# marcin-ochman/modular-slam

Measured on AMD Instinct MI355X. Metric: ORB keypoints extracted+matched /sec, 640×480 RGB-D, 1/2/4/8 GPU; HBM GB/s vs roofline, higher is better.
Workload: dtype u8

## Files before the change

### modular-slam_amd/csrc/k_quadtree.hip

```cpp
#include "common.hpp"
#include <cstdlib>

namespace mslam
{

constexpr int QT = 512;
constexpr int kSmallKp = 512, kSmallQT = 256;
constexpr int kMidKp = 1024, kMidQT = 512;
constexpr int kLdsKp = 2048;
constexpr int kMaxCellsPerLevel = 2048;
constexpr int kBigNodes = 4096;
constexpr int kBigKp = 12288;
constexpr int kBigMinPixels = 400000;
constexpr int kMaxInitNodes = 64;
constexpr int kMaxPasses = 40;

struct Scan
{
    uint32_t wsum[QT / 64];
};

__device__ __forceinline__ uint32_t wave_incl_scan(uint32_t v)
{
    int x = (int)v;
    x += __builtin_amdgcn_update_dpp(0, x, 0x111, 0xF, 0xF, true);
    x += __builtin_amdgcn_update_dpp(0, x, 0x112, 0xF, 0xF, true);
    x += __builtin_amdgcn_update_dpp(0, x, 0x114, 0xF, 0xE, true);
    x += __builtin_amdgcn_update_dpp(0, x, 0x118, 0xF, 0xC, true);
    x += __builtin_amdgcn_update_dpp(0, x, 0x142, 0xA, 0xF, true);
    x += __builtin_amdgcn_update_dpp(0, x, 0x143, 0xC, 0xF, true);
    return (uint32_t)x;
}

template <int NT>
__device__ __forceinline__ uint32_t block_excl_scan(uint32_t v, Scan& s, uint32_t& total)
{
    const int lane = threadIdx.x & 63, wave = threadIdx.x >> 6;
    const uint32_t inc = wave_incl_scan(v);
    if(lane == 63)
        s.wsum[wave] = inc;
    __syncthreads();
    uint32_t base = 0, tot = 0;
#pragma unroll
    for(int w = 0; w < NT / 64; ++w)
    {
        const uint32_t x = s.wsum[w];
        if(w < wave)
// ... 131 lines not shown
    __syncthreads();
    if(tid == 0)
    {
        uint32_t n0 = 0;
        for(int i = 0; i < n_init; ++i)
        {
            init_pos[i] = n0;
            if(init_cnt[i] != 0)
            {
                const int ix = i % lv.nxg, iy = i / lv.nxg;
                nodes[n0] = pack_node((int)(lv.delta_x * ix), (int)(lv.delta_y * iy), (int)(lv.delta_x * (ix + 1)),
                                      (int)(lv.delta_y * (iy + 1)));
                ncnt[n0] = (idx_t)init_cnt[i];
                ++n0;
            }
        }
        sh_n = n0;
    }
    __syncthreads();
    for(uint32_t k = tid; k < N; k += NT)
    {
        const uint32_t idx = kp_node[k];
        if(idx != kNoNode)
            kp_node[k] = (idx_t)init_pos[idx];
    }
    uint32_t n = sh_n;
    __syncthreads();

    const float sf = lv.scale;
    const float min_size_f = (float)a.min_size;
    bool converged = false;
    for(int pass = 0; pass < kMaxPasses && n > 0; ++pass)
    {
        for(uint32_t pos = tid; pos < n; pos += NT)
        {
            int bx, by, ex, ey;
            unpack_node(nodes[pos], bx, by, ex, ey);
            const unsigned area = (unsigned)((ex - bx) * (ey - by));
            const bool keep = (uint32_t)ncnt[pos] == 1u || __fmul_rn(__fmul_rn((float)area, sf), sf) <= min_size_f;
            ninfo[pos] = keep ? 0u : 1u;
            if(!keep)
                S::cc_zero(cc, pos);
        }
        __syncthreads();
        for(uint32_t k = tid; k < N; k += NT)
        {
            const uint32_t pos = kp_node[k];
            if(pos == kNoNode || !(ninfo[pos] & 1u))
                continue;
            int bx, by, ex, ey;
            unpack_node(nodes[pos], bx, by, ex, ey);
            const int cx = bx + ((ex - bx + 1) >> 1), cy = by + ((ey - by + 1) >> 1);
            const uint32_t p = cand[k];
            S::cc_add(cc, pos, (cx <= kp_x(p) ? 1 : 0) + (cy <= kp_y(p) ? 2 : 0));
        }
        __syncthreads();
        uint32_t D = 0, U = 0;
        for(uint32_t base = 0; base < n; base += NT)
        {
            const uint32_t pos = base + tid;
            uint32_t nchild = 0, und = 0, mask = 0, div = 0;
            if(pos < n)
            {
                div = ninfo[pos] & 1u;
                if(div)
                {
                    mask = (S::cc_get(cc, pos, 0) ? 1u : 0u) | (S::cc_get(cc, pos, 1) ? 2u : 0u) |
                           (S::cc_get(cc, pos, 2) ? 4u : 0u) | (S::cc_get(cc, pos, 3) ? 8u : 0u);
                    nchild = (uint32_t)__popc(mask);
                }
                else
                    und = 1;
            }
            uint32_t totD, totU, exD, exU;
            block_excl_scan2<NT>(nchild, und, scan, scan2, exD, exU, totD, totU);
            if(pos < n)
            {
// ... 87 lines not shown
        a.sel_cnt[slot] = n;
    return true;
}

template <int NT>
__device__ __forceinline__ uint32_t quad_cell_offsets(const uint32_t* ccnt, int n_cells, uint32_t* cell_off, Scan& scan)
{
    const int tid = threadIdx.x;
    uint32_t running = 0;
    for(int base = 0; base < n_cells; base += NT)
    {
        const int i = base + tid;
        const uint32_t v = i < n_cells ? ccnt[i] : 0u;
        uint32_t tot;
        const uint32_t ex = block_excl_scan<NT>(v, scan, tot);
        if(i < n_cells)
            cell_off[i] = running + ex;
        running += tot;
    }
    if(tid == 0)
        cell_off[n_cells] = running;
    __syncthreads();
    return running;
}

__device__ __forceinline__ int quad_class(uint32_t N, int n_cells, unsigned classes)
{
    if((classes & 1u) && N <= (uint32_t)kSmallKp && n_cells <= 2 * kSmallKp - 1)
        return 0;
    if((classes & 2u) && N <= (uint32_t)kMidKp && n_cells <= 2 * kMidKp - 1)
        return 1;
    return 2;
}
template <int KP, int NT, int CLS>
__global__ __launch_bounds__(NT) __attribute__((amdgpu_waves_per_eu(CLS == 2 ? 4 : 8))) void k_quadtree(Geometry g, QuadArgs a, unsigned big_levels)
{
    __shared__ Scan scan, scan2;
    __shared__ uint32_t l_cand[KP];
    __shared__ uint2 l_nodes_a[KP], l_nodes_b[KP];
    __shared__ uint32_t l_cc[KP * 2];
    __shared__ uint16_t l_kp_node[KP], l_ncnt_a[KP], l_ncnt_b[KP], l_nbase[KP];
    __shared__ uint8_t l_ninfo[KP];
    __shared__ uint32_t init_cnt[kMaxInitNodes];
    __shared__ uint32_t init_pos[kMaxInitNodes];
    __shared__ uint32_t sh_n;
    constexpr int kCellsFit = 2 * KP - 1;
    static_assert(CLS != 2 || kCellsFit >= kMaxCellsPerLevel, "cell offsets must fit");
    const unsigned classes = big_levels >> 30;
    uint32_t* cell_off = reinterpret_cast<uint32_t*>(l_nodes_b);

    const int level = (int)((blockIdx.x + blockIdx.y) % (unsigned)g.n_levels);
    const size_t frame = blockIdx.y + g.frame0;
    const LevelGeom& lv = g.lv[level];
    const int tid = threadIdx.x;
    const size_t slot = frame * g.n_levels + level;
    const size_t cap = (size_t)a.cand_cap;
    uint32_t* cand = a.cand + slot * cap;
    uint32_t* sel = a.sel + slot * cap;

    const int n_cells = lv.n_cells;
    if(n_cells > kCellsFit)
        return;
    const uint32_t* ccnt = a.cell_cnt + frame * g.n_cells + lv.cell_base;
    const uint32_t N = quad_cell_offsets<NT>(ccnt, n_cells, cell_off, scan);
    if(quad_class(N, n_cells, classes) != CLS)
        return;
    if(N > (uint32_t)a.cand_cap)
    {
        if(tid == 0)
        {
            atomicOr(a.flags, kFlagCandOverflow);
            a.cand_cnt[slot] = 0;
            a.sel_cnt[slot] = 0;
        }
        return;
    }
    if(tid == 0)
        a.cand_cnt[slot] = N;
    if(N == 0)
    {
        if(tid == 0)
            a.sel_cnt[slot] = 0;
        return;
    }
    if(N <= (uint32_t)KP)
        quad_run<LdsStore, NT>(g, a, lv, frame, slot, tid, N, n_cells, cell_off, l_cand, cand, l_kp_node, l_nodes_a, l_nodes_b,
                               l_ncnt_a, l_ncnt_b, l_ninfo, l_nbase, l_cc, l_cc, sel, scan, scan2, init_cnt, init_pos, sh_n);
    else if((big_levels >> level) & 1u)
        return;
    else
        quad_run<GlobalStore, NT>(g, a, lv, frame, slot, tid, N, n_cells, cell_off, cand, cand, a.kp_node + slot * cap,
                                  a.nodes_a + slot * cap, a.nodes_b + slot * cap, a.ncnt_a + slot * cap,
                                  a.ncnt_b + slot * cap, a.ninfo + slot * cap, a.best + slot * cap,
                                  a.child_cnt + slot * cap * 4, a.best + slot * cap, sel, scan, scan2, init_cnt, init_pos,
                                  sh_n);
}

__global__ __launch_bounds__(QT) void k_quadtree_big(Geometry g, QuadArgs a, unsigned big_levels)
{
    extern __shared__ __attribute__((aligned(16))) uint8_t big_lds[];
    __shared__ Scan scan, scan2;
    __shared__ uint32_t init_cnt[kMaxInitNodes];
    __shared__ uint32_t init_pos[kMaxInitNodes];
    __shared__ uint32_t sh_n;
    uint2* l_nodes_a = reinterpret_cast<uint2*>(big_lds);
    uint2* l_nodes_b = l_nodes_a + kBigNodes;
    uint32_t* l_cc = reinterpret_cast<uint32_t*>(l_nodes_b + kBigNodes);
    uint16_t* l_kp_node = reinterpret_cast<uint16_t*>(l_cc + 2 * kBigNodes);
    uint16_t* l_ncnt_a = l_kp_node + kBigKp;
    uint16_t* l_ncnt_b = l_ncnt_a + kBigNodes;
    uint16_t* l_nbase = l_ncnt_b + kBigNodes;
    uint8_t* l_ninfo = reinterpret_cast<uint8_t*>(l_nbase + kBigNodes);
    static_assert(kBigNodes * sizeof(uint2) >= (kMaxCellsPerLevel + 1) * sizeof(uint32_t), "cell offsets must fit");
    uint32_t* cell_off = reinterpret_cast<uint32_t*>(l_nodes_b);

    int level = 0;
    {
        unsigned m = big_levels;
        const unsigned which = (blockIdx.x + blockIdx.y) % gridDim.x;
        for(unsigned i = 0; i < which; ++i)
            m &= m - 1;
        level = __ffs((int)m) - 1;
    }
    const size_t frame = blockIdx.y + g.frame0;
    const LevelGeom& lv = g.lv[level];
    const int tid = threadIdx.x;
    const size_t slot = frame * g.n_levels + level;
    const size_t cap = (size_t)a.cand_cap;
    uint32_t* cand = a.cand + slot * cap;
    uint32_t* sel = a.sel + slot * cap;
    const int n_cells = lv.n_cells;
    const uint32_t* ccnt = a.cell_cnt + frame * g.n_cells + lv.cell_base;
    const uint32_t N = quad_cell_offsets<QT>(ccnt, n_cells, cell_off, scan);
    if(N <= (uint32_t)kLdsKp || N > (uint32_t)a.cand_cap)
        return;
    bool done = false;
    if(N <= (uint32_t)kBigKp)
        done = quad_run<BigStore, QT>(g, a, lv, frame, slot, tid, N, n_cells, cell_off, cand, cand, l_kp_node, l_nodes_a, l_nodes_b,
                                  l_ncnt_a, l_ncnt_b, l_ninfo, l_nbase, l_cc, l_cc, sel, scan, scan2, init_cnt, init_pos, sh_n);
    if(!done)
    {
        __syncthreads();
        quad_cell_offsets<QT>(ccnt, n_cells, cell_off, scan);
        quad_run<GlobalStore, QT>(g, a, lv, frame, slot, tid, N, n_cells, cell_off, cand, cand, a.kp_node + slot * cap,
                              a.nodes_a + slot * cap, a.nodes_b + slot * cap, a.ncnt_a + slot * cap,
                              a.ncnt_b + slot * cap, a.ninfo + slot * cap, a.best + slot * cap,
                              a.child_cnt + slot * cap * 4, a.best + slot * cap, sel, scan, scan2, init_cnt, init_pos,
                              sh_n);
    }
}

void launch_quadtree(const Geometry& g, const QuadArgs& a, int frame0, int n_frames, hipStream_t s)
{
    dim3 grid(g.n_levels, n_frames);
    Geometry gg = g;
    gg.frame0 = frame0;
    unsigned big_levels = 0;
    for(int l = 0; l < g.n_levels; ++l)
        if(g.lv[l].w * g.lv[l].h > kBigMinPixels)
            big_levels |= 1u << l;
    static const unsigned classes_env = [] { const char* e = getenv("MSLAM_HIP_QUAD_CLASSES"); return e ? (unsigned)atoi(e) & 3u : 3u; }();
    const unsigned classes = n_frames < 8 ? 0u : classes_env;
    const unsigned bl = big_levels | (classes << 30);
    hipLaunchKernelGGL((k_quadtree<kLdsKp, QT, 2>), grid, dim3(QT), 0, s, gg, a, bl);
    if(classes & 2u)
        hipLaunchKernelGGL((k_quadtree<kMidKp, kMidQT, 1>), grid, dim3(kMidQT), 0, s, gg, a, bl);
    if(classes & 1u)
        hipLaunchKernelGGL((k_quadtree<kSmallKp, kSmallQT, 0>), grid, dim3(kSmallQT), 0, s, gg, a, bl);
    if(big_levels != 0)
    {
        constexpr size_t lds = (size_t)kBigNodes * (8 + 8 + 8 + 2 + 2 + 2 + 1) + (size_t)kBigKp * 2;
        static const bool attr = [] {
            return hipFuncSetAttribute((const void*)k_quadtree_big, hipFuncAttributeMaxDynamicSharedMemorySize, (int)lds) == hipSuccess;
        }();
        (void)attr;
        hipLaunchKernelGGL(k_quadtree_big, dim3((unsigned)__builtin_popcount(big_levels), n_frames), dim3(QT), lds, s, gg, a,
                           big_levels);
    }
}

}
```

### include/mslam_hip.h

```cpp
#ifndef MSLAM_HIP_H_
#define MSLAM_HIP_H_

#include <stddef.h>
#include <stdint.h>

#ifdef __cplusplus
extern "C" {
#endif

#define MSLAM_HIP_ABI_VERSION 5

enum
{
    MSLAM_HIP_OK = 0,
    MSLAM_HIP_E_INVALID = 1,
    MSLAM_HIP_E_RUNTIME = 2,
    MSLAM_HIP_E_CAPACITY = 3,
    MSLAM_HIP_E_NO_VOCABULARY = 4,
    MSLAM_HIP_E_FORMAT = 5,
    MSLAM_HIP_E_NO_MODEL = 6
};

typedef struct mslam_hip_ctx mslam_hip_ctx;

// ... 259 lines not shown
} mslam_hip_track_result;
int mslam_hip_track(mslam_hip_ctx* ctx, const uint8_t* desc, const float* xy, int n, const uint16_t* depth, int width,
                    int height, float factor, double fx, double fy, double cx, double cy, int ref_id,
                    const int32_t* vote_ids, int n_vote, double ratio, int iterations, double reprojection_error,
                    uint64_t seed, int use_extrinsic_guess, const double* rvec, const double* tvec,
                    int min_matched_points , int new_keyframe_min_landmarks , int new_id ,
                    double z_max , mslam_hip_track_result* out, int32_t* vote_counts ,
                    int32_t* pair_from, int32_t* pair_to, uint8_t* inliers, int pair_stride,
                    int32_t* entry_src, int32_t* entry_kp, int entry_capacity);

typedef mslam_hip_track_result mslam_hip_track_window_result;
int mslam_hip_track_window(mslam_hip_ctx* ctx, const uint8_t* desc, const float* xy, const int32_t* n, int stride,
                           const uint16_t* depth, int S, int width, int height, float factor, double fx, double fy, double cx,
                           double cy, int ref_id, const int32_t* vote_ids, int n_vote, int ref_vote_pos, double ratio,
                           int iterations, double reprojection_error, uint64_t seed, int use_extrinsic_guess,
                           const double* rvec, const double* tvec, int min_matched_points, int new_keyframe_min_landmarks,
                           int new_id, double z_max, mslam_hip_track_window_result* out , int* first_event,
                           int32_t* vote_counts , int32_t* entry_src, int32_t* entry_kp,
                           int entry_capacity);
int mslam_hip_track_window_dev(mslam_hip_ctx* ctx, int first_frame, int n_frames, double fx, double fy, double cx, double cy,
                               int ref_id, const int32_t* vote_ids, int n_vote, int ref_vote_pos, double ratio, int iterations,
                               double reprojection_error, uint64_t seed, int use_extrinsic_guess, const double* rvec,
                               const double* tvec, int min_matched_points, int new_keyframe_min_landmarks, int new_id,
                               double z_max, mslam_hip_track_window_result* out , int* first_event,
                               int32_t* vote_counts, int32_t* entry_src, int32_t* entry_kp, int entry_capacity);

enum
{
    MSLAM_HIP_DBG_PYRAMID = 0,
    MSLAM_HIP_DBG_BLURRED = 1,
    MSLAM_HIP_DBG_CANDIDATES = 2,
    MSLAM_HIP_DBG_SELECTED = 3,
    MSLAM_HIP_DBG_CELLS = 4,
    MSLAM_HIP_DBG_FORMS = 5
};
int mslam_hip_level_geometry(mslam_hip_ctx* ctx, int* widths, int* heights, float* scales);
int mslam_hip_debug_read(mslam_hip_ctx* ctx, int what, int frame, int level, void* dst, size_t dst_bytes,
                         size_t* n_items);

int mslam_hip_debug_counts(mslam_hip_ctx* ctx, int what, int32_t* out, int n_frames);

int mslam_hip_copy_to_host(mslam_hip_ctx* ctx, void* dst_host, const void* src_dev, size_t bytes);

int mslam_hip_set_profiling(mslam_hip_ctx* ctx, int enable);
int mslam_hip_get_stage_times(mslam_hip_ctx* ctx, const char** names, float* ms, int cap, int* n);

#ifdef __cplusplus
}
#endif
#endif
```

### modular-slam_amd/__init__.py

```python
import ctypes as C
import os
import subprocess

import numpy as np

_HERE = os.path.dirname(os.path.abspath(__file__))
LIB_PATH = os.path.join(_HERE, "libmslam_hip.so")

OK, E_INVALID, E_RUNTIME, E_CAPACITY, E_NO_VOCABULARY, E_FORMAT, E_NO_MODEL = range(7)
DBG_PYRAMID, DBG_BLURRED, DBG_CANDIDATES, DBG_SELECTED, DBG_CELLS, DBG_FORMS = range(6)
MATCHER_AUTO, MATCHER_POPCOUNT = 0, 1
DETECTOR_DISTRIBUTED, DETECTOR_CV_ORB = 0, 1
BOW_ASSIGN_TREE, BOW_ASSIGN_FLAT = 0, 1
CV_ORDER_LIBSTDCXX, CV_ORDER_RASTER = 0, 1

ABI_SYMBOLS = [
    "mslam_hip_default_params", "mslam_hip_abi_version", "mslam_hip_create", "mslam_hip_destroy",
    "mslam_hip_last_error", "mslam_hip_sync", "mslam_hip_detect", "mslam_hip_detect_batch_dev",
    "mslam_hip_get_batch_view", "mslam_hip_match", "mslam_hip_match_knn2", "mslam_hip_match_batch_dev",
    "mslam_hip_bow_load", "mslam_hip_bow_info", "mslam_hip_bow_words", "mslam_hip_bow_transform",
    "mslam_hip_bow_score", "mslam_hip_bow_db_add", "mslam_hip_bow_db_query", "mslam_hip_bow_db_clear",
    "mslam_hip_bow_batch_dev", "mslam_hip_get_bow_view", "mslam_hip_bow_cross_score_dev", "mslam_hip_level_geometry", "mslam_hip_debug_read",
    "mslam_hip_set_profiling", "mslam_hip_get_stage_times", "mslam_hip_copy_to_host", "mslam_hip_backproject", "mslam_hip_backproject_batch_dev",
    "mslam_hip_get_points_view", "mslam_hip_set_matcher", "mslam_hip_get_matcher",
    "mslam_hip_bow_pack_dev", "mslam_hip_bow_cross_score_packed_dev", "mslam_hip_debug_counts",
    "mslam_hip_last_match_kernel",
    "mslam_hip_join_matcher", "mslam_hip_bow_db_remove", "mslam_hip_bow_set_assignment",
    "mslam_hip_bow_db_reserve", "mslam_hip_bow_db_size", "mslam_hip_qlz_decompress",
    "mslam_hip_pnp_ransac", "mslam_hip_pnp_batch_dev", "mslam_hip_get_pnp_view", "mslam_hip_pnp_set_confidence", "mslam_hip_pack_batch_dev", "mslam_hip_packed_capacity",
    "mslam_hip_set_cv_keypoint_order", "mslam_hip_pnp_min_mse", "mslam_hip_pnp_min_mse_batch_dev",
    "mslam_hip_kf_add", "mslam_hip_kf_add_from_batch_dev", "mslam_hip_kf_remove", "mslam_hip_kf_clear", "mslam_hip_kf_size",
    "mslam_hip_kf_reserve", "mslam_hip_kf_read", "mslam_hip_relocalize",
    "mslam_hip_kf_visible", "mslam_hip_track", "mslam_hip_track_window", "mslam_hip_track_window_dev",
    "mslam_hip_kf_add_ids", "mslam_hip_kf_read_ids", "mslam_hip_kf_covisible", "mslam_hip_kf_union", "mslam_hip_kf_union_dev",
    "mslam_hip_match_guided_knn2", "mslam_hip_match_guided", "mslam_hip_set_guided_match", "mslam_hip_get_guided_match",
    "mslam_hip_bundle_adjust", "mslam_hip_bundle_adjust_global", "mslam_hip_kf_update_world",
]


class MslamHipError(RuntimeError):
    def __init__(self, code, msg):
        super().__init__("mslam_hip error %d: %s" % (code, msg))
        self.code = code
# ... 690 lines not shown
        n = self.params.n_levels
        w = (C.c_int * 16)()
        h = (C.c_int * 16)()
        s = (C.c_float * 16)()
        self._chk(self.L.mslam_hip_level_geometry(self._h, w, h, s))
        return list(w[:n]), list(h[:n]), np.array(s[:n], np.float32)

    def debug_image(self, what, frame, level):
        w, h, _ = self.level_geometry()
        out = np.empty((h[level], w[level]), np.uint8)
        n = C.c_size_t(0)
        self._chk(self.L.mslam_hip_debug_read(self._h, what, frame, level, _p(out), C.c_size_t(out.size), C.byref(n)))
        return out

    def debug_keypoints(self, what, frame, level):
        out = np.empty((self.params.max_candidates, 3), np.float32)
        n = C.c_size_t(0)
        self._chk(self.L.mslam_hip_debug_read(self._h, what, frame, level, _p(out), C.c_size_t(out.nbytes),
                                              C.byref(n)))
        return out[:n.value].copy()

    def debug_cells(self, level):
        out = np.empty((2048, 6), np.int32)
        n = C.c_size_t(0)
        self._chk(self.L.mslam_hip_debug_read(self._h, DBG_CELLS, 0, level, _p(out), C.c_size_t(out.nbytes),
                                              C.byref(n)))
        return out[:n.value].copy()

    def debug_forms(self):
        out = np.zeros(2, np.int32)
        n = C.c_size_t(0)
        self._chk(self.L.mslam_hip_debug_read(self._h, DBG_FORMS, 0, 0, _p(out), C.c_size_t(out.nbytes), C.byref(n)))
        return int(out[0]), int(out[1])

    def debug_counts(self, what, n_frames):
        out = np.zeros((max(n_frames, 1), self.params.n_levels), np.int32)
        self._chk(self.L.mslam_hip_debug_counts(self._h, int(what), _p(out), int(out.shape[0])))
        return out[:n_frames]

    def set_profiling(self, enable):
        self._chk(self.L.mslam_hip_set_profiling(self._h, int(enable)))

    def stage_times(self, cap=256):
        names = (C.c_char_p * cap)()
        ms = (C.c_float * cap)()
        n = C.c_int(0)
        self._chk(self.L.mslam_hip_get_stage_times(self._h, names, ms, cap, C.byref(n)))
        return [(names[i].decode(), ms[i]) for i in range(n.value)]


def qlz_decompress(data, n_packets, capacity=None):
    src = np.frombuffer(bytes(data), np.uint8)
    cap = capacity if capacity is not None else 10000 * n_packets + 16
    dst = np.empty(max(cap, 1), np.uint8)
    n = C.c_size_t(0)
    L = lib()
    L.mslam_hip_qlz_decompress.argtypes = [C.c_void_p, C.c_size_t, C.c_uint32, C.c_void_p, C.c_size_t, C.POINTER(C.c_size_t)]
    rc = L.mslam_hip_qlz_decompress(_p(src), src.size, int(n_packets), _p(dst), dst.size, C.byref(n))
    if rc != OK:
        raise MslamHipError(rc, "qlz_decompress failed")
    return dst[:n.value].tobytes()


class RgbFrame:

    def __init__(self, data, width, height):
# ... 396 lines not shown
```

### modular-slam_amd/csrc/api.hip

```cpp
#include "context.hpp"

#include <cfloat>
#include <climits>
#include <cmath>
#include <cstdio>
#include <cstring>
#include <cstdlib>
#include <algorithm>

using namespace mslam;

static thread_local std::string g_create_error;

#define ENTER(c)                                                                                                       \
    do                                                                                                                 \
    {                                                                                                                  \
        if(!(c))                                                                                                       \
            return MSLAM_HIP_E_INVALID;                                                                                \
        MSLAM_CHK(c, hipSetDevice((c)->p.device));                                                                     \
    } while(0)

static inline int cv_round_f(float v) { return (int)lrintf(v); }
static inline int cv_floor_f(float v)
{
// ... 148 lines not shown
                cd.cw = (int16_t)(max_x - min_x);
                cd.ch = (int16_t)(max_y - min_y);
                cd.x0 = (int16_t)min_x;
                cd.y0 = (int16_t)min_y;
                cd.ox = (int16_t)(j * kCell);
                cd.oy = (int16_t)(i * kCell);
                c->cells.push_back(cd);
            }
        }
        lv.n_cells = (int)c->cells.size() - lv.cell_base;
        if(lv.n_cells > 2048)
            return fail(c, MSLAM_HIP_E_INVALID, "more than 2048 FAST cells on one level");

        lv.bsx = (lv.w + 3) / 4;

        const int min_x = kBorder, max_x = lv.w - kBorder, min_y = kBorder, max_y = lv.h - kBorder;
        const double ratio = (double)(max_x - min_x) / (max_y - min_y);
        if(ratio > 1)
        {
            lv.nxg = (int)std::round(ratio);
            lv.nyg = 1;
            lv.delta_x = (double)(max_x - min_x) / lv.nxg;
            lv.delta_y = max_y - min_y;
        }
        else
        {
            lv.nxg = 1;
            lv.nyg = (int)std::round(1 / ratio);
            lv.delta_x = max_x - min_y;
            lv.delta_y = (double)(max_y - min_y) / lv.nyg;
        }
        if(lv.nxg * lv.nyg > 64)
            return fail(c, MSLAM_HIP_E_INVALID, "aspect ratio beyond 64:1 is not supported");
    }
    g.slab = offset + 256;
    g.n_cells = (int)c->cells.size();
    return MSLAM_HIP_OK;
}

static int build_geometry_cv(mslam_hip_ctx* c)
{
    const mslam_hip_params& p = c->p;
    Geometry& g = c->geom;
    g.n_levels = p.n_levels;
    g.W = p.width;
    g.H = p.height;
    g.blur_tiled = 0;
    const double sf = (double)p.scale_factor;
    unsigned offset = 0;
    c->cells.clear();
    for(int l = 0; l < p.n_levels; ++l)
    {
        LevelGeom& lv = g.lv[l];
        lv = LevelGeom{};
        lv.scale = (float)std::pow(sf, (double)l);
        const float inv = 1.0f / lv.scale;
        lv.w = cv_round_f((float)p.width * inv);
        lv.h = cv_round_f((float)p.height * inv);
        if(lv.w < 16 || lv.h < 16)
            return fail(c, MSLAM_HIP_E_INVALID, "pyramid level " + std::to_string(l) + " is smaller than 16 px");
        if(lv.w > 4095 || lv.h > 4095)
            return fail(c, MSLAM_HIP_E_INVALID, "frames larger than 4095 px per side are not supported");
        lv.pitch = (lv.w + kTileW - 1) & ~(kTileW - 1);
        lv.offset = (int)offset;
        offset += ((unsigned)lv.pitch * ((lv.h + kTileH - 1) & ~(kTileH - 1)) + 255u) & ~255u;
        lv.bw = lv.w - 2 * kBorder;
        lv.bh = lv.h - 2 * kBorder;
        lv.bsx = (lv.w + 3) / 4;
    }
    g.slab = offset + 256;
    g.n_cells = 0;
    const float factor = (float)(1.0 / sf);
    float desired = (float)p.n_features * (1 - factor) / (1 - (float)std::pow((double)factor, (double)p.n_levels));
    int sum = 0;
    for(int l = 0; l < p.n_levels - 1; ++l)
    {
        c->cv_quota[l] = cv_round_f(desired);
        sum += c->cv_quota[l];
        desired *= factor;
    }
    c->cv_quota[p.n_levels - 1] = std::max(p.n_features - sum, 0);
    return MSLAM_HIP_OK;
}

static void exact_axis(int ssize, int dsize, std::vector<int32_t>& ofs, std::vector<uint32_t>& coef, int& dmin, int& dmax)
{
    const double scale = 1.0 / ((double)dsize / (double)ssize);
// ... 1435 lines not shown
                                       (size_t)n * 4, hipMemcpyDeviceToHost));
            for(uint32_t i = 0; i < n; ++i)
            {
                out[3 * i] += (float)kBorder;
                out[3 * i + 1] += (float)kBorder;
                out[3 * i + 2] = resp[i];
            }
        }
        return MSLAM_HIP_OK;
    }
    if(what == MSLAM_HIP_DBG_CELLS && c->p.detector == MSLAM_HIP_DETECTOR_DISTRIBUTED)
    {
        *n_items = (size_t)lv.n_cells;
        if(dst_bytes < (size_t)lv.n_cells * 24)
            return fail(c, MSLAM_HIP_E_CAPACITY, "debug_read: buffer too small");
        int32_t* out = static_cast<int32_t*>(dst);
        for(int i = 0; i < lv.n_cells; ++i)
        {
            const CellDesc& cd = c->cells[(size_t)lv.cell_base + i];
            const int32_t rec[6] = {cd.x0, cd.y0, cd.cw, cd.ch, cd.ox, cd.oy};
            std::memcpy(out + 6 * i, rec, sizeof(rec));
        }
        return MSLAM_HIP_OK;
    }
    if(what == MSLAM_HIP_DBG_FORMS)
    {
        *n_items = 2;
        if(dst_bytes < 8)
            return fail(c, MSLAM_HIP_E_CAPACITY, "debug_read: buffer too small");
        const int32_t rec[2] = {c->fused_levels, c->geom.blur_tiled};
        std::memcpy(dst, rec, sizeof(rec));
        return MSLAM_HIP_OK;
    }
    return fail(c, MSLAM_HIP_E_INVALID, "debug_read: unknown item");
}

int mslam_hip_debug_counts(mslam_hip_ctx* c, int what, int32_t* out, int n_frames)
{
    ENTER(c);
    if(c->p.width == 0 || !out || n_frames < 1 || (what != MSLAM_HIP_DBG_CANDIDATES && what != MSLAM_HIP_DBG_SELECTED))
        return fail(c, MSLAM_HIP_E_INVALID, "debug_counts: bad argument");
    MSLAM_CHK(c, hipStreamSynchronize(c->stream));
    const int rows = std::min(n_frames, std::max(c->n_last, 1));
    MSLAM_CHK(c, hipMemcpy(out, what == MSLAM_HIP_DBG_CANDIDATES ? c->quad.cand_cnt : c->quad.sel_cnt,
                           (size_t)rows * c->geom.n_levels * 4, hipMemcpyDeviceToHost));
    return MSLAM_HIP_OK;
}

int mslam_hip_copy_to_host(mslam_hip_ctx* c, void* dst_host, const void* src_dev, size_t bytes)
{
    ENTER(c);
    if(!dst_host || !src_dev)
        return fail(c, MSLAM_HIP_E_INVALID, "copy_to_host: null pointer");
    MSLAM_CHK(c, hipStreamSynchronize(c->stream_m));
    MSLAM_CHK(c, hipStreamSynchronize(c->stream));
    MSLAM_CHK(c, hipMemcpy(dst_host, src_dev, bytes, hipMemcpyDeviceToHost));
    return MSLAM_HIP_OK;
}

int mslam_hip_set_profiling(mslam_hip_ctx* c, int enable)
{
    if(!c)
        return MSLAM_HIP_E_INVALID;
    c->profiling = enable == 1;
    c->inplace_timing = enable == 2;
    c->timers_used = 0;
// ... 28 lines not shown
```

### modular-slam_amd/csrc/common.hpp

```cpp
#pragma once
#include <hip/hip_runtime.h>
#include <cstdint>
#include <cstddef>

namespace mslam
{

constexpr int kMaxLevels = 16;
constexpr int kBorder = 19;
constexpr int kCell = 64;
constexpr int kOverlap = 6;
constexpr int kCellCap = 1024;

constexpr size_t al256(size_t x) { return (x + 255) & ~(size_t)255; }

struct LevelGeom
{
    int w, h;
    int pitch;
    int offset;
    float scale;
    int bw, bh;
    int cell_base;
    int n_cells;
    int bsx;
    int nxg, nyg;
    double delta_x, delta_y;
};

struct Geometry
{
    int n_levels;
    int W, H;
    int n_cells;
    int frame0;
    unsigned slab;
    int blur_tiled;
    LevelGeom lv[kMaxLevels];
};

#ifndef MSLAM_TILE_W
#define MSLAM_TILE_W 64
#endif
constexpr int kTileW = MSLAM_TILE_W, kTileH = 128 / kTileW;
constexpr int kTileWLog = kTileW == 64 ? 6 : kTileW == 32 ? 5 : 4, kTileHLog = 7 - kTileWLog;
static_assert(kTileW == 16 || kTileW == 32 || kTileW == 64, "tile width");
__host__ __device__ __forceinline__ unsigned tiled_off(unsigned pitch, int x, int y)
{
    return (unsigned)(y >> kTileHLog) * (pitch * (unsigned)kTileH) + (unsigned)(x >> kTileWLog) * 128u +
           (unsigned)(y & (kTileH - 1)) * (unsigned)kTileW + (unsigned)(x & (kTileW - 1));
}
template <class P>
__device__ __forceinline__ P lds_ptr(uint32_t off)
{
#if defined(__HIP_DEVICE_COMPILE__)
    return (P)off;
#else
    return (P)(uintptr_t)off;
#endif
}
// ... 35 lines not shown
    const uint32_t* ycoef;
    int frame0, n_frames;
    int quads;
    float inv_quads;
    int R;
    int need_mask;
    int exact;
};
void launch_resize_col(const ResizeColArgs& a, hipStream_t s);
void launch_fast(const uint8_t* d_pyr, const Geometry& g, const CellDesc* d_cells, uint32_t* d_cell_cnt,
                 uint32_t* d_cell_kp, int ini_thr, int min_thr, int frame0, int n_frames, hipStream_t s);
void launch_denorm_selfcheck(uint32_t* d_out, hipStream_t s);
struct QuadArgs
{
    const uint32_t* cell_cnt;
    const uint32_t* cell_kp;
    uint32_t* cand;
    uint32_t* cand_cnt;
    uint32_t* sel;
    uint32_t* sel_cnt;
    uint32_t* kp_node;
    uint2* nodes_a;
    uint2* nodes_b;
    uint32_t* ncnt_a;
    uint32_t* ncnt_b;
    uint32_t* child_cnt;
    uint32_t* ninfo;
    uint32_t* best;
    uint32_t* flags;
    int cand_cap;
    unsigned min_size;
};
void launch_quadtree(const Geometry& g, const QuadArgs& a, int frame0, int n_frames, hipStream_t s);
struct BlurK
{
    uint32_t ta[3], tb[4], tc[4];
    uint32_t t01, t23, t45, t6;
};
BlurK make_blur_k();
struct GrayBlurArgs
{
    const uint8_t* bgr;
    uint8_t* pyr;
    uint8_t* blur;
    int W, H, pitch;
    unsigned slab;
    int n_frames, frame0;
    int quads;
    float inv_quads;
    int wide;
    int k6;
    int waves_per_xcd;
    int blur_tiled;
    BlurK bk;
};
void launch_gray_blur(const GrayBlurArgs& a, hipStream_t s);
struct ResizeBlurArgs
{
    uint8_t* pyr;
    uint8_t* blur;
    unsigned slab;
    int src_off, sh, spitch, dst_off, dw, dh, dpitch;
    const uint4* qt;
    const int32_t* yofs;
    const uint32_t* ycoef;
    int frame0, n_frames;
// ... 172 lines not shown
```

Baseline: 647.8 million.

## Classify quadtree pairs up front, walk large pairs persistently, exit converged passes early

Adds a small classify kernel that sums per-level cell counts once per (frame, level) pair and records candidate counts and overflow flags. The size-class kernels and the big kernel then read that count instead of each recomputing it and early-exiting. The large class becomes a persistent grid sized to a multiple of the CU count, with each block iterating over the pairs assigned to it, which avoids launching many blocks that immediately exit. The distribution pass also breaks out early via a block-wide ballot when no node divides, saving the keypoint scatter and the remaining passes. This adds an extra launch and serializes the large pairs within each block.

```diff
diff --git a/modular-slam_amd/csrc/k_quadtree.hip b/modular-slam_amd/csrc/k_quadtree.hip
--- a/modular-slam_amd/csrc/k_quadtree.hip
+++ b/modular-slam_amd/csrc/k_quadtree.hip
@@ -210,6 +210,7 @@
     bool converged = false;
     for(int pass = 0; pass < kMaxPasses && n > 0; ++pass)
     {
+        bool divides = false;
         for(uint32_t pos = tid; pos < n; pos += NT)
         {
             int bx, by, ex, ey;
@@ -218,9 +219,24 @@
             const bool keep = (uint32_t)ncnt[pos] == 1u || __fmul_rn(__fmul_rn((float)area, sf), sf) <= min_size_f;
             ninfo[pos] = keep ? 0u : 1u;
             if(!keep)
+            {
                 S::cc_zero(cc, pos);
-        }
+                divides = true;
+            }
+        }
+        const bool wave_divides = __ballot(divides) != 0;
+        if((threadIdx.x & 63) == 0)
+            scan.wsum[threadIdx.x >> 6] = wave_divides ? 1u : 0u;
         __syncthreads();
+        uint32_t any_divides = 0;
+#pragma unroll
+        for(int w = 0; w < NT / 64; ++w)
+            any_divides |= scan.wsum[w];
+        if(!any_divides)
+        {
+            converged = true;
+            break;
+        }
         for(uint32_t k = tid; k < N; k += NT)
         {
             const uint32_t pos = kp_node[k];
@@ -374,8 +390,40 @@
         return 1;
     return 2;
 }
-template <int KP, int NT, int CLS>
-__global__ __launch_bounds__(NT) __attribute__((amdgpu_waves_per_eu(CLS == 2 ? 4 : 8))) void k_quadtree(Geometry g, QuadArgs a, unsigned big_levels)
+
+constexpr int kClassifyNT = 256;
+__global__ __launch_bounds__(kClassifyNT) void k_quadtree_classify(Geometry g, QuadArgs a, unsigned n_pairs)
+{
+    const unsigned pair = blockIdx.x * (unsigned)(kClassifyNT / 64) + (threadIdx.x >> 6);
+    if(pair >= n_pairs)
+        return;
+    const int lane = threadIdx.x & 63;
+    const int level = (int)(pair % (unsigned)g.n_levels);
+    const size_t frame = pair / (unsigned)g.n_levels + g.frame0;
+    const LevelGeom& lv = g.lv[level];
+    const uint32_t* ccnt = a.cell_cnt + frame * g.n_cells + lv.cell_base;
+    uint32_t v = 0;
+    for(int i = lane; i < lv.n_cells; i += 64)
+        v += ccnt[i];
+    const uint32_t N = (uint32_t)__builtin_amdgcn_readlane((int)wave_incl_scan(v), 63);
+    if(lane != 0)
+        return;
+    const size_t slot = frame * g.n_levels + level;
+    if(N > (uint32_t)a.cand_cap)
+    {
+        atomicOr(a.flags, kFlagCandOverflow);
+        a.cand_cnt[slot] = 0;
+        a.sel_cnt[slot] = 0;
+        return;
+    }
+    a.cand_cnt[slot] = N;
+    if(N == 0)
+        a.sel_cnt[slot] = 0;
+}
+
+template <int KP, int NT, int CLS, bool WALK>
+__global__ __launch_bounds__(NT) __attribute__((amdgpu_waves_per_eu(CLS == 2 ? 4 : 8))) void k_quadtree(Geometry g, QuadArgs a, unsigned big_levels,
+                                                                                                       unsigned n_pairs)
 {
     __shared__ Scan scan, scan2;
     __shared__ uint32_t l_cand[KP];
@@ -388,54 +436,94 @@
     __shared__ uint32_t sh_n;
     constexpr int kCellsFit = 2 * KP - 1;
     static_assert(CLS != 2 || kCellsFit >= kMaxCellsPerLevel, "cell offsets must fit");
+    static_assert(CLS == 2 || !WALK, "only the large instance walks");
+    constexpr bool kCounted = CLS != 2 || WALK;
     const unsigned classes = big_levels >> 30;
     uint32_t* cell_off = reinterpret_cast<uint32_t*>(l_nodes_b);
-
-    const int level = (int)((blockIdx.x + blockIdx.y) % (unsigned)g.n_levels);
-    const size_t frame = blockIdx.y + g.frame0;
-    const LevelGeom& lv = g.lv[level];
     const int tid = threadIdx.x;
-    const size_t slot = frame * g.n_levels + level;
-    const size_t cap = (size_t)a.cand_cap;
-    uint32_t* cand = a.cand + slot * cap;
-    uint32_t* sel = a.sel + slot * cap;
-
-    const int n_cells = lv.n_cells;
-    if(n_cells > kCellsFit)
-        return;
-    const uint32_t* ccnt = a.cell_cnt + frame * g.n_cells + lv.cell_base;
-    const uint32_t N = quad_cell_offsets<NT>(ccnt, n_cells, cell_off, scan);
-    if(quad_class(N, n_cells, classes) != CLS)
-        return;
-    if(N > (uint32_t)a.cand_cap)
-    {
-        if(tid == 0)
-        {
-            atomicOr(a.flags, kFlagCandOverflow);
-            a.cand_cnt[slot] = 0;
-            a.sel_cnt[slot] = 0;
-        }
-        return;
-    }
-    if(tid == 0)
-        a.cand_cnt[slot] = N;
-    if(N == 0)
-    {
-        if(tid == 0)
-            a.sel_cnt[slot] = 0;
-        return;
-    }
-    if(N <= (uint32_t)KP)
-        quad_run<LdsStore, NT>(g, a, lv, frame, slot, tid, N, n_cells, cell_off, l_cand, cand, l_kp_node, l_nodes_a, l_nodes_b,
-                               l_ncnt_a, l_ncnt_b, l_ninfo, l_nbase, l_cc, l_cc, sel, scan, scan2, init_cnt, init_pos, sh_n);
-    else if((big_levels >> level) & 1u)
-        return;
+
+    const auto run_pair = [&](int level, size_t frame) {
+        const LevelGeom& lv = g.lv[level];
+        const size_t slot = frame * g.n_levels + level;
+        const size_t cap = (size_t)a.cand_cap;
+        uint32_t* cand = a.cand + slot * cap;
+        uint32_t* sel = a.sel + slot * cap;
+
+        const int n_cells = lv.n_cells;
+        const uint32_t* ccnt = a.cell_cnt + frame * g.n_cells + lv.cell_base;
+        uint32_t N;
+        if(kCounted)
+        {
+            N = a.cand_cnt[slot];
+            if(N == 0 || quad_class(N, n_cells, classes) != CLS)
+                return;
+            quad_cell_offsets<NT>(ccnt, n_cells, cell_off, scan);
+        }
+        else
+        {
+            N = quad_cell_offsets<NT>(ccnt, n_cells, cell_off, scan);
+            if(N > (uint32_t)a.cand_cap)
+            {
+                if(tid == 0)
+                {
+                    atomicOr(a.flags, kFlagCandOverflow);
+                    a.cand_cnt[slot] = 0;
+                    a.sel_cnt[slot] = 0;
+                }
+                return;
+            }
+            if(tid == 0)
+                a.cand_cnt[slot] = N;
+            if(N == 0)
+            {
+                if(tid == 0)
+                    a.sel_cnt[slot] = 0;
+                return;
+            }
+        }
+        if(CLS != 2 || N <= (uint32_t)KP)
+            quad_run<LdsStore, NT>(g, a, lv, frame, slot, tid, N, n_cells, cell_off, l_cand, cand, l_kp_node, l_nodes_a, l_nodes_b,
+                                   l_ncnt_a, l_ncnt_b, l_ninfo, l_nbase, l_cc, l_cc, sel, scan, scan2, init_cnt, init_pos, sh_n);
+        else if((big_levels >> level) & 1u)
+            return;
+        else
+            quad_run<GlobalStore, NT>(g, a, lv, frame, slot, tid, N, n_cells, cell_off, cand, cand, a.kp_node + slot * cap,
+                                      a.nodes_a + slot * cap, a.nodes_b + slot * cap, a.ncnt_a + slot * cap,
+                                      a.ncnt_b + slot * cap, a.ninfo + slot * cap, a.best + slot * cap,
+                                      a.child_cnt + slot * cap * 4, a.best + slot * cap, sel, scan, scan2, init_cnt, init_pos,
+                                      sh_n);
+    };
+
+    const unsigned L = (unsigned)g.n_levels;
+    if(WALK)
+    {
+        const unsigned G = gridDim.x;
+        const unsigned lane = threadIdx.x & 63u;
+        for(unsigned first = blockIdx.x; first < n_pairs; first += 64u * G)
+        {
+            const unsigned p = first + lane * G;
+            bool mine = false;
+            if(p < n_pairs)
+            {
+                const unsigned fr = p / L, level = (p % L + fr + fr * L / G) % L;
+                const uint32_t N = a.cand_cnt[((size_t)fr + g.frame0) * L + level];
+                int n_cells = 0;
+                for(unsigned l = 0; l < L; ++l)
+                    n_cells = l == level ? g.lv[l].n_cells : n_cells;
+                mine = N != 0 && quad_class(N, n_cells, classes) == 2;
+            }
+            for(unsigned long long todo = __ballot(mine); todo != 0; todo &= todo - 1)
+            {
+                const unsigned q = first + (unsigned)__builtin_ctzll(todo) * G, fr = q / L;
+                run_pair((int)((q % L + fr + fr * L / G) % L), (size_t)fr + g.frame0);
+                __syncthreads();
+            }
+        }
+    }
     else
-        quad_run<GlobalStore, NT>(g, a, lv, frame, slot, tid, N, n_cells, cell_off, cand, cand, a.kp_node + slot * cap,
-                                  a.nodes_a + slot * cap, a.nodes_b + slot * cap, a.ncnt_a + slot * cap,
-                                  a.ncnt_b + slot * cap, a.ninfo + slot * cap, a.best + slot * cap,
-                                  a.child_cnt + slot * cap * 4, a.best + slot * cap, sel, scan, scan2, init_cnt, init_pos,
-                                  sh_n);
+    {
+        run_pair((int)((blockIdx.x + blockIdx.y) % L), (size_t)blockIdx.y + g.frame0);
+    }
 }
 
 __global__ __launch_bounds__(QT) void k_quadtree_big(Geometry g, QuadArgs a, unsigned big_levels)
@@ -473,9 +561,10 @@
     uint32_t* sel = a.sel + slot * cap;
     const int n_cells = lv.n_cells;
     const uint32_t* ccnt = a.cell_cnt + frame * g.n_cells + lv.cell_base;
-    const uint32_t N = quad_cell_offsets<QT>(ccnt, n_cells, cell_off, scan);
-    if(N <= (uint32_t)kLdsKp || N > (uint32_t)a.cand_cap)
+    const uint32_t N = a.cand_cnt[slot];
+    if(N <= (uint32_t)kLdsKp)
         return;
+    quad_cell_offsets<QT>(ccnt, n_cells, cell_off, scan);
     bool done = false;
     if(N <= (uint32_t)kBigKp)
         done = quad_run<BigStore, QT>(g, a, lv, frame, slot, tid, N, n_cells, cell_off, cand, cand, l_kp_node, l_nodes_a, l_nodes_b,
@@ -492,9 +581,26 @@
     }
 }
 
+static unsigned quad_walk_grid()
+{
+    static unsigned cus[64];
+    int dev = 0;
+    if(hipGetDevice(&dev) != hipSuccess || dev < 0 || dev >= 64)
+        dev = 0;
+    if(cus[dev] == 0)
+    {
+        int n = 0;
+        if(hipDeviceGetAttribute(&n, hipDeviceAttributeMultiprocessorCount, dev) != hipSuccess || n <= 0)
+            n = 256;
+        cus[dev] = (unsigned)n;
+    }
+    return 4 * cus[dev];
+}
+
 void launch_quadtree(const Geometry& g, const QuadArgs& a, int frame0, int n_frames, hipStream_t s)
 {
     dim3 grid(g.n_levels, n_frames);
+    const unsigned n_pairs = (unsigned)g.n_levels * (unsigned)n_frames;
     Geometry gg = g;
     gg.frame0 = frame0;
     unsigned big_levels = 0;
@@ -504,11 +610,20 @@
     static const unsigned classes_env = [] { const char* e = getenv("MSLAM_HIP_QUAD_CLASSES"); return e ? (unsigned)atoi(e) & 3u : 3u; }();
     const unsigned classes = n_frames < 8 ? 0u : classes_env;
     const unsigned bl = big_levels | (classes << 30);
-    hipLaunchKernelGGL((k_quadtree<kLdsKp, QT, 2>), grid, dim3(QT), 0, s, gg, a, bl);
-    if(classes & 2u)
-        hipLaunchKernelGGL((k_quadtree<kMidKp, kMidQT, 1>), grid, dim3(kMidQT), 0, s, gg, a, bl);
-    if(classes & 1u)
-        hipLaunchKernelGGL((k_quadtree<kSmallKp, kSmallQT, 0>), grid, dim3(kSmallQT), 0, s, gg, a, bl);
+    if(classes == 0)
+        hipLaunchKernelGGL((k_quadtree<kLdsKp, QT, 2, false>), grid, dim3(QT), 0, s, gg, a, bl, n_pairs);
+    else
+    {
+        hipLaunchKernelGGL(k_quadtree_classify, dim3((n_pairs + kClassifyNT / 64 - 1) / (kClassifyNT / 64)), dim3(kClassifyNT), 0, s,
+                           gg, a, n_pairs);
+        if(classes & 2u)
+            hipLaunchKernelGGL((k_quadtree<kMidKp, kMidQT, 1, false>), grid, dim3(kMidQT), 0, s, gg, a, bl, n_pairs);
+        if(classes & 1u)
+            hipLaunchKernelGGL((k_quadtree<kSmallKp, kSmallQT, 0, false>), grid, dim3(kSmallQT), 0, s, gg, a, bl, n_pairs);
+        const unsigned walk = quad_walk_grid();
+        hipLaunchKernelGGL((k_quadtree<kLdsKp, QT, 2, true>), dim3(walk < n_pairs ? walk : n_pairs), dim3(QT), 0, s, gg, a, bl,
+                           n_pairs);
+    }
     if(big_levels != 0)
     {
         constexpr size_t lds = (size_t)kBigNodes * (8 + 8 + 8 + 2 + 2 + 2 + 1) + (size_t)kBigKp * 2;
```

New measurement: 656.7 million (median of 4 runs). Within noise of the previous version (+1.4%).

## Add direct implicit-quadtree kernel for small pyramid levels in ORB distribution

Applied to the files above, without the earlier changes.

Adds a k_quadtree_direct kernel that, for levels whose full quadtree depth fits in a small fixed slot table, computes each keypoint's quadtree path at once and counts per node with LDS atomics. It then resolves leaves level by level and picks the best keypoint per leaf with atomicMax, replacing the iterative node-splitting passes. The existing kernel skips those levels when N fits, and the class-split launches are dropped when every level is direct. It adds an extra kernel launch and must reproduce the original node-splitting and ordering semantics exactly, which is a correctness risk.

```diff
diff --git a/include/mslam_hip.h b/include/mslam_hip.h
--- a/include/mslam_hip.h
+++ b/include/mslam_hip.h
@@ -315,7 +315,8 @@
     MSLAM_HIP_DBG_CANDIDATES = 2,
     MSLAM_HIP_DBG_SELECTED = 3,
     MSLAM_HIP_DBG_CELLS = 4,
-    MSLAM_HIP_DBG_FORMS = 5
+    MSLAM_HIP_DBG_FORMS = 5,
+    MSLAM_HIP_DBG_QUAD_DIRECT = 6
 };
 int mslam_hip_level_geometry(mslam_hip_ctx* ctx, int* widths, int* heights, float* scales);
 int mslam_hip_debug_read(mslam_hip_ctx* ctx, int what, int frame, int level, void* dst, size_t dst_bytes,
diff --git a/modular-slam_amd/__init__.py b/modular-slam_amd/__init__.py
--- a/modular-slam_amd/__init__.py
+++ b/modular-slam_amd/__init__.py
@@ -8,7 +8,8 @@
 LIB_PATH = os.path.join(_HERE, "libmslam_hip.so")
 
 OK, E_INVALID, E_RUNTIME, E_CAPACITY, E_NO_VOCABULARY, E_FORMAT, E_NO_MODEL = range(7)
-DBG_PYRAMID, DBG_BLURRED, DBG_CANDIDATES, DBG_SELECTED, DBG_CELLS, DBG_FORMS = range(6)
+DBG_PYRAMID, DBG_BLURRED, DBG_CANDIDATES, DBG_SELECTED, DBG_CELLS, DBG_FORMS, DBG_QUAD_DIRECT = range(7)
+QUAD_DIRECT_MAX_CANDIDATES = 1024
 MATCHER_AUTO, MATCHER_POPCOUNT = 0, 1
 DETECTOR_DISTRIBUTED, DETECTOR_CV_ORB = 0, 1
 BOW_ASSIGN_TREE, BOW_ASSIGN_FLAT = 0, 1
@@ -765,6 +766,12 @@
         n = C.c_size_t(0)
         self._chk(self.L.mslam_hip_debug_read(self._h, DBG_FORMS, 0, 0, _p(out), C.c_size_t(out.nbytes), C.byref(n)))
         return int(out[0]), int(out[1])
+
+    def debug_quad_direct_levels(self):
+        out = np.zeros(1, np.uint32)
+        n = C.c_size_t(0)
+        self._chk(self.L.mslam_hip_debug_read(self._h, DBG_QUAD_DIRECT, 0, 0, _p(out), C.c_size_t(out.nbytes), C.byref(n)))
+        return [bool((int(out[0]) >> l) & 1) for l in range(self.params.n_levels)]
 
     def debug_counts(self, what, n_frames):
         out = np.zeros((max(n_frames, 1), self.params.n_levels), np.int32)
diff --git a/modular-slam_amd/csrc/api.hip b/modular-slam_amd/csrc/api.hip
--- a/modular-slam_amd/csrc/api.hip
+++ b/modular-slam_amd/csrc/api.hip
@@ -204,6 +204,7 @@
         }
         if(lv.nxg * lv.nyg > 64)
             return fail(c, MSLAM_HIP_E_INVALID, "aspect ratio beyond 64:1 is not supported");
+        lv.qdepth = quad_depth_bound(lv, (unsigned)p.min_node_area);
     }
     g.slab = offset + 256;
     g.n_cells = (int)c->cells.size();
@@ -225,6 +226,7 @@
     {
         LevelGeom& lv = g.lv[l];
         lv = LevelGeom{};
+        lv.qdepth = -1;
         lv.scale = (float)std::pow(sf, (double)l);
         const float inv = 1.0f / lv.scale;
         lv.w = cv_round_f((float)p.width * inv);
@@ -1726,6 +1728,15 @@
         std::memcpy(dst, rec, sizeof(rec));
         return MSLAM_HIP_OK;
     }
+    if(what == MSLAM_HIP_DBG_QUAD_DIRECT)
+    {
+        *n_items = 1;
+        if(dst_bytes < 4)
+            return fail(c, MSLAM_HIP_E_CAPACITY, "debug_read: buffer too small");
+        const uint32_t m = c->p.detector == MSLAM_HIP_DETECTOR_DISTRIBUTED ? quad_direct_levels(c->geom) : 0u;
+        std::memcpy(dst, &m, sizeof(m));
+        return MSLAM_HIP_OK;
+    }
     return fail(c, MSLAM_HIP_E_INVALID, "debug_read: unknown item");
 }
 
diff --git a/modular-slam_amd/csrc/common.hpp b/modular-slam_amd/csrc/common.hpp
--- a/modular-slam_amd/csrc/common.hpp
+++ b/modular-slam_amd/csrc/common.hpp
@@ -26,6 +26,7 @@
     int bsx;
     int nxg, nyg;
     double delta_x, delta_y;
+    int qdepth;
 };
 
 struct Geometry
@@ -127,6 +128,8 @@
     unsigned min_size;
 };
 void launch_quadtree(const Geometry& g, const QuadArgs& a, int frame0, int n_frames, hipStream_t s);
+int quad_depth_bound(const LevelGeom& lv, unsigned min_size);
+unsigned quad_direct_levels(const Geometry& g);
 struct BlurK
 {
     uint32_t ta[3], tb[4], tc[4];
diff --git a/modular-slam_amd/csrc/k_quadtree.hip b/modular-slam_amd/csrc/k_quadtree.hip
--- a/modular-slam_amd/csrc/k_quadtree.hip
+++ b/modular-slam_amd/csrc/k_quadtree.hip
@@ -1,4 +1,5 @@
 #include "common.hpp"
+#include <algorithm>
 #include <cstdlib>
 
 namespace mslam
@@ -13,6 +14,7 @@
 constexpr int kBigKp = 12288;
 constexpr int kBigMinPixels = 400000;
 constexpr int kMaxInitNodes = 64;
+constexpr int kDirectKp = 1024, kDirectQT = 256, kDirectSlots = 1365, kDirectMaxDepth = 10;
 constexpr int kMaxPasses = 40;
 
 struct Scan
@@ -375,7 +377,7 @@
     return 2;
 }
 template <int KP, int NT, int CLS>
-__global__ __launch_bounds__(NT) __attribute__((amdgpu_waves_per_eu(CLS == 2 ? 4 : 8))) void k_quadtree(Geometry g, QuadArgs a, unsigned big_levels)
+__global__ __launch_bounds__(NT) __attribute__((amdgpu_waves_per_eu(CLS == 2 ? 4 : 8))) void k_quadtree(Geometry g, QuadArgs a, unsigned big_levels, unsigned direct_levels)
 {
     __shared__ Scan scan, scan2;
     __shared__ uint32_t l_cand[KP];
@@ -405,6 +407,8 @@
         return;
     const uint32_t* ccnt = a.cell_cnt + frame * g.n_cells + lv.cell_base;
     const uint32_t N = quad_cell_offsets<NT>(ccnt, n_cells, cell_off, scan);
+    if(((direct_levels >> level) & 1u) && N <= (uint32_t)kDirectKp)
+        return;
     if(quad_class(N, n_cells, classes) != CLS)
         return;
     if(N > (uint32_t)a.cand_cap)
@@ -492,6 +496,261 @@
     }
 }
 
+template <int SLOTS>
+struct DirectTable
+{
+    uint32_t cnt[(SLOTS + 1) / 2];
+    uint32_t best[SLOTS];
+    uint8_t flag[SLOTS];
+};
+
+__device__ __forceinline__ uint32_t direct_block_start(uint32_t n_init, int d) { return n_init * (((1u << (2 * d)) - 1u) / 3u); }
+
+template <int KP, int SLOTS, int NT>
+__global__ __launch_bounds__(NT) __attribute__((amdgpu_waves_per_eu(8))) void k_quadtree_direct(Geometry g, QuadArgs a, unsigned direct_levels)
+{
+    constexpr int PER = KP / NT;
+    static_assert(KP % NT == 0 && KP == kDirectKp, "instance shape");
+    __shared__ Scan scan;
+    __shared__ uint32_t l_cand[KP];
+    __shared__ DirectTable<SLOTS> t;
+    __shared__ uint32_t tot[2 * (kDirectMaxDepth + 2)];
+
+    const int level = (int)((blockIdx.x + blockIdx.y) % (unsigned)g.n_levels);
+    if(!((direct_levels >> level) & 1u))
+        return;
+    const size_t frame = blockIdx.y + g.frame0;
+    const LevelGeom& lv = g.lv[level];
+    const int tid = threadIdx.x;
+    const size_t slot = frame * g.n_levels + level;
+    const size_t cap = (size_t)a.cand_cap;
+    uint32_t* g_cand = a.cand + slot * cap;
+    uint32_t* sel = a.sel + slot * cap;
+    const int D = lv.qdepth;
+    const uint32_t n_init = (uint32_t)(lv.nxg * lv.nyg);
+    const uint32_t n_slots = direct_block_start(n_init, D + 1);
+
+    for(uint32_t i = tid; i < (n_slots + 1) / 2; i += NT)
+        t.cnt[i] = 0;
+    for(uint32_t i = tid; i < n_slots; i += NT)
+        t.flag[i] = 0;
+    if(tid < 2 * (kDirectMaxDepth + 2))
+        tot[tid] = 0;
+
+    const int n_cells = lv.n_cells;
+    uint32_t* cell_off = t.best;
+    const uint32_t* ccnt = a.cell_cnt + frame * g.n_cells + lv.cell_base;
+    const uint32_t N = quad_cell_offsets<NT>(ccnt, n_cells, cell_off, scan);
+    if(N > (uint32_t)KP)
+        return;
+    if(N > (uint32_t)a.cand_cap)
+    {
+        if(tid == 0)
+        {
+            atomicOr(a.flags, kFlagCandOverflow);
+            a.cand_cnt[slot] = 0;
+            a.sel_cnt[slot] = 0;
+        }
+        return;
+    }
+    if(tid == 0)
+        a.cand_cnt[slot] = N;
+    if(N == 0)
+    {
+        if(tid == 0)
+            a.sel_cnt[slot] = 0;
+        return;
+    }
+
+    const uint32_t* ckp = a.cell_kp + (frame * g.n_cells + lv.cell_base) * (size_t)kCellCap;
+    const float sf = lv.scale;
+    const float min_size_f = (float)a.min_size;
+    uint32_t path[PER];
+#pragma unroll
+    for(int i = 0; i < PER; ++i)
+    {
+        const uint32_t k = (uint32_t)(tid + i * NT);
+        path[i] = ~0u;
+        if(k >= N)
+            continue;
+        int lo = 0, hi = n_cells - 1;
+        while(lo < hi)
+        {
+            const int mid = (lo + hi + 1) >> 1;
+            if(cell_off[mid] <= k)
+                lo = mid;
+            else
+                hi = mid - 1;
+        }
+        const uint32_t p = ckp[(size_t)lo * kCellCap + (k - cell_off[lo])];
+        l_cand[k] = p;
+        g_cand[k] = p;
+        const int x = kp_x(p), y = kp_y(p);
+        const unsigned ix = (unsigned)((double)(float)x / lv.delta_x);
+        const unsigned iy = (unsigned)((double)(float)y / lv.delta_y);
+        const unsigned idx = ix + iy * (unsigned)lv.nxg;
+        if(idx >= n_init)
+            continue;
+        int bx = (int)(lv.delta_x * ix), by = (int)(lv.delta_y * iy);
+        int ex = (int)(lv.delta_x * (ix + 1)), ey = (int)(lv.delta_y * (iy + 1));
+        uint32_t q = idx;
+        int d = 0;
+        for(;;)
+        {
+            const uint32_t s = direct_block_start(n_init, d) + q;
+            atomicAdd(&t.cnt[s >> 1], 1u << (16 * (s & 1u)));
+            const unsigned area = (unsigned)((ex - bx) * (ey - by));
+            if(__fmul_rn(__fmul_rn((float)area, sf), sf) <= min_size_f || d == D)
+            {
+                t.flag[s] = 1;
+                break;
+            }
+            const int cx = bx + ((ex - bx + 1) >> 1), cy = by + ((ey - by + 1) >> 1);
+            const bool right = cx <= x, low = cy <= y;
+            bx = right ? cx : bx, ex = right ? ex : cx;
+            by = low ? cy : by, ey = low ? ey : cy;
+            q = (q << 2) | (right ? 1u : 0u) | (low ? 2u : 0u);
+            ++d;
+        }
+        path[i] = ((uint32_t)d << 24) | q;
+    }
+    __syncthreads();
+
+    for(int d = 0; d <= D; ++d)
+    {
+        const uint32_t start = direct_block_start(n_init, d), n_d = n_init << (2 * d);
+        const uint32_t pstart = direct_block_start(n_init, d > 0 ? d - 1 : 0);
+        uint32_t kd = 0, md = 0;
+        for(uint32_t base = 0; base < n_d; base += NT)
+        {
+            const uint32_t q = base + tid;
+            bool keep = false, open = false;
+            if(q < n_d)
+            {
+                const uint32_t s = start + q, ps = pstart + (q >> 2);
+                const uint32_t c = (t.cnt[s >> 1] >> (16 * (s & 1u))) & 0xFFFFu;
+                const uint32_t pc = d > 0 ? (t.cnt[ps >> 1] >> (16 * (ps & 1u))) & 0xFFFFu : 2u;
+                const bool real = c > 0 && pc >= 2;
+                keep = real && (c == 1 || t.flag[s] != 0);
+                open = real && !keep;
+                t.flag[s] = keep ? 1 : open ? 2 : 0;
+                t.best[s] = 0;
+            }
+            kd += (uint32_t)__popcll(__ballot(keep));
+            md += (uint32_t)__popcll(__ballot(open));
+        }
+        if((tid & 63) == 0 && (kd | md) != 0)
+        {
+            atomicAdd(&tot[2 * d], kd);
+            atomicAdd(&tot[2 * d + 1], md);
+        }
+    }
+    __syncthreads();
+    int P = 1;
+    while(tot[2 * P] + tot[2 * P + 1] != tot[2 * P - 1])
+        ++P;
+    const int top = P < D ? P : D;
+
+#pragma unroll
+    for(int i = 0; i < PER; ++i)
+    {
+        if(path[i] == ~0u)
+            continue;
+        const uint32_t k = (uint32_t)(tid + i * NT);
+        const int dk = (int)(path[i] >> 24);
+        const uint32_t q = path[i] & 0xFFFFFFu;
+        const int last = dk < top ? dk : top;
+        uint32_t leaf = 0;
+        for(int d = 0; d <= last; ++d)
+        {
+            leaf = direct_block_start(n_init, d) + (q >> (2 * (dk - d)));
+            if(t.flag[leaf] == 1)
+                break;
+        }
+        atomicMax(&t.best[leaf], ((uint32_t)kp_score(l_cand[k]) << 24) | (0xFFFFFFu - k));
+    }
+    __syncthreads();
+
+    const uint32_t n_entries = direct_block_start(n_init, top + 1);
+    const uint32_t per = (n_entries + NT - 1) / NT;
+    const uint32_t e0 = (uint32_t)tid * per, e1 = e0 + per < n_entries ? e0 + per : n_entries;
+    auto entry_slot = [&](uint32_t e, bool& is_leaf) {
+        int d = top;
+        uint32_t n_d = n_init << (2 * d);
+        while(e >= n_d)
+        {
+            e -= n_d;
+            --d;
+            n_d >>= 2;
+        }
+        const uint32_t bits = 2u * (uint32_t)d, low_mask = (1u << bits) - 1u;
+        uint32_t i0 = e >> bits;
+        if(d & 1)
+            i0 = n_init - 1u - i0;
+        const uint32_t s = direct_block_start(n_init, d) + ((i0 << bits) | ((e ^ 0x33333333u) & low_mask));
+        const uint32_t f = t.flag[s];
+        is_leaf = f == 1 || (f == 2 && d == P);
+        return s;
+    };
+    uint32_t mine = 0;
+    for(uint32_t e = e0; e < e1; ++e)
+    {
+        bool is_leaf;
+        entry_slot(e, is_leaf);
+        mine += is_leaf ? 1u : 0u;
+    }
+    uint32_t n_leaves;
+    uint32_t r = block_excl_scan<NT>(mine, scan, n_leaves);
+    for(uint32_t e = e0; e < e1 && mine != 0; ++e)
+    {
+        bool is_leaf;
+        const uint32_t s = entry_slot(e, is_leaf);
+        if(is_leaf)
+            sel[r++] = l_cand[0xFFFFFFu - (t.best[s] & 0xFFFFFFu)];
+    }
+    if(tid == 0)
+        a.sel_cnt[slot] = n_leaves;
+}
+
+unsigned quad_direct_levels(const Geometry& g)
+{
+    const char* env = getenv("MSLAM_HIP_QUAD_DIRECT");
+    const bool on = !env || atoi(env) != 0;
+    unsigned m = 0;
+    for(int l = 0; on && l < g.n_levels; ++l)
+    {
+        const LevelGeom& lv = g.lv[l];
+        if(lv.qdepth < 0 || lv.qdepth > kDirectMaxDepth || lv.n_cells + 1 > kDirectSlots)
+            continue;
+        const long long slots = (long long)lv.nxg * lv.nyg * (((1ll << (2 * (lv.qdepth + 1))) - 1) / 3);
+        if(slots <= kDirectSlots)
+            m |= 1u << l;
+    }
+    return m;
+}
+
+int quad_depth_bound(const LevelGeom& lv, unsigned min_size)
+{
+    int dx = 0, dy = 0;
+    for(int iy = 0; iy < lv.nyg; ++iy)
+        for(int ix = 0; ix < lv.nxg; ++ix)
+        {
+            dx = std::max(dx, (int)(lv.delta_x * (ix + 1)) - (int)(lv.delta_x * ix));
+            dy = std::max(dy, (int)(lv.delta_y * (iy + 1)) - (int)(lv.delta_y * iy));
+        }
+    for(int d = 0; d <= 15; ++d)
+    {
+        const unsigned area = (unsigned)(dx * dy);
+        const float scaled = (float)area * lv.scale;
+        if(scaled * lv.scale <= (float)min_size)
+            return d;
+        if(dx <= 1 && dy <= 1)
+            break;
+        dx = (dx + 1) >> 1, dy = (dy + 1) >> 1;
+    }
+    return -1;
+}
+
 void launch_quadtree(const Geometry& g, const QuadArgs& a, int frame0, int n_frames, hipStream_t s)
 {
     dim3 grid(g.n_levels, n_frames);
@@ -502,13 +761,17 @@
         if(g.lv[l].w * g.lv[l].h > kBigMinPixels)
             big_levels |= 1u << l;
     static const unsigned classes_env = [] { const char* e = getenv("MSLAM_HIP_QUAD_CLASSES"); return e ? (unsigned)atoi(e) & 3u : 3u; }();
-    const unsigned classes = n_frames < 8 ? 0u : classes_env;
+    const unsigned direct = quad_direct_levels(g);
+    const bool all_direct = direct == (g.n_levels >= 32 ? ~0u : (1u << g.n_levels) - 1u);
+    const unsigned classes = n_frames < 8 || all_direct ? 0u : classes_env;
     const unsigned bl = big_levels | (classes << 30);
-    hipLaunchKernelGGL((k_quadtree<kLdsKp, QT, 2>), grid, dim3(QT), 0, s, gg, a, bl);
+    if(direct != 0)
+        hipLaunchKernelGGL((k_quadtree_direct<kDirectKp, kDirectSlots, kDirectQT>), grid, dim3(kDirectQT), 0, s, gg, a, direct);
+    hipLaunchKernelGGL((k_quadtree<kLdsKp, QT, 2>), grid, dim3(QT), 0, s, gg, a, bl, direct);
     if(classes & 2u)
-        hipLaunchKernelGGL((k_quadtree<kMidKp, kMidQT, 1>), grid, dim3(kMidQT), 0, s, gg, a, bl);
+        hipLaunchKernelGGL((k_quadtree<kMidKp, kMidQT, 1>), grid, dim3(kMidQT), 0, s, gg, a, bl, direct);
     if(classes & 1u)
-        hipLaunchKernelGGL((k_quadtree<kSmallKp, kSmallQT, 0>), grid, dim3(kSmallQT), 0, s, gg, a, bl);
+        hipLaunchKernelGGL((k_quadtree<kSmallKp, kSmallQT, 0>), grid, dim3(kSmallQT), 0, s, gg, a, bl, direct);
     if(big_levels != 0)
     {
         constexpr size_t lds = (size_t)kBigNodes * (8 + 8 + 8 + 2 + 2 + 2 + 1) + (size_t)kBigKp * 2;
```

Result: faster. 643.1 million before, 668.3 million after, median of 6 (+3.9%).
